# pierluigiferrari/ssd_keras

Measured on AMD Instinct MI355X. Metric: images/sec SSD300 fwd+decode @batch32, higher is better.
Workload: dtype f32 (decode, threshold, TF-style f32 NMS, top-k); bf16 conv backbone; 1 GPU; SSD300 VGG-16 inference (mode='inference': forward + DecodeDetections), 21 classes, batch 32 per GPU, conf 0.01 / NMS 0.45 / top-200, random-init weights, synthetic 300x300x3 uint8-range images; per_gpu_batch=32, global_batch=32, conv_dtype=bf16, parallelism=replicas x1, launch=hip_graph (forward + DecodeDetections captured once, replayed per step), decode_stream=same stream; DecodeDetections reads the head outputs directly (no y_pred in HBM)

## Files before the change

### ssd_keras_amd/csrc/ssdhip_conv64.hip

```cpp
#include <hip/hip_runtime.h>
#include <stdint.h>
#include <stdlib.h>

#include <type_traits>

#include "ssdhip.h"
#include "ssdhip_math.h"

#ifndef SSDHIP_C64_ABLATE
#define SSDHIP_C64_ABLATE 0
#endif

namespace ssdhip {

typedef unsigned short bf16_t;
typedef __bf16 bf16x8 __attribute__((ext_vector_type(8)));
typedef float f32x16 __attribute__((ext_vector_type(16)));
typedef int i32x4 __attribute__((ext_vector_type(4)));

#ifdef SSDHIP_PROFILE
__device__ unsigned long long g_prof64[32];
#define C64_PROF_DECL long long _pt = clock64(); long long _pa[8] = {0, 0, 0, 0, 0, 0, 0, 0}; int _pn = 0;
#define C64_PROF_MARK(i) { const long long _t = clock64(); _pa[i] += _t - _pt; _pt = _t; }
#define C64_PROF_TILE ++_pn;
#define C64_PROF_FLUSH(base) if (lane == 0) { for (int _i = 0; _i < 8; ++_i) atomicAdd(&g_prof64[(base) + _i], (unsigned long long)_pa[_i]); atomicAdd(&g_prof64[(base) + 8], (unsigned long long)_pn); }
#else
#define C64_PROF_DECL
#define C64_PROF_MARK(i)
#define C64_PROF_TILE
#define C64_PROF_FLUSH(base)
#endif

#ifndef SSDHIP_C64_NLOAD
#define SSDHIP_C64_NLOAD 1
#endif
constexpr int C64_NLOAD = SSDHIP_C64_NLOAD;
constexpr int C64_THREADS = (4 + C64_NLOAD) * 64;
constexpr int C64_NPROD = 3;
constexpr int C64_FRONT_THREADS = (4 + C64_NPROD) * 64;
constexpr int C64_WBYTES = 9 * 64 * 128;
constexpr int C64_STAGE = 0;
constexpr int c64_halo_bytes(int cs) { return ((9 * (2 * (64 >> cs) + 2) * ((1 << cs) + 2) + 63) / 64) * 1024; }
constexpr int C64_PATCH1 = 1600;
constexpr int C64_PATCH = ((C64_NPROD * C64_PATCH1 + 1023) / 1024) * 1024;
constexpr int C64_WREG_BYTES = 1024;
constexpr int c64_lds_bytes(int cs, int nb, bool front = false, bool wreg = false) {
    return (wreg ? C64_WREG_BYTES : C64_WBYTES) + nb * c64_halo_bytes(cs) + C64_STAGE + (front ? C64_PATCH : 0);
}

struct C64Params {
    const bf16_t* x;
    const bf16_t* w;
    const bf16_t* bias;
    bf16_t* y;
    int B, H, W, Cout, relu;
    int HT, WT, n_slices, tiles;
    int Ho, Wo;
    int x_bytes, w_bytes;
    const bf16_t* x3;
    const bf16_t* w1;
    const bf16_t* b1;
    int prio;
    int xcd_pairs;
    bf16_t* y2;
};

__device__ __forceinline__ u32 c64_f2bf_rn(float f) {
    const u32 u = __float_as_uint(f);
    if ((u & 0x7fffffffu) > 0x7f800000u) return (u >> 16) | 0x40u;
    return (u + 0x7fffu + ((u >> 16) & 1u)) >> 16;
}

#if defined(__HIP_DEVICE_COMPILE__)
typedef __bf16 c64_bf16x2 __attribute__((ext_vector_type(2)));
typedef float c64_f32x2 __attribute__((ext_vector_type(2)));
__device__ __forceinline__ u32 c64_pack2(float a, float b) {
    const c64_f32x2 v = {a, b};
    return __builtin_bit_cast(u32, __builtin_convertvector(v, c64_bf16x2));
}
__device__ __forceinline__ float c64_max_with_lane_xor1(float v) {
    float r;
    asm("s_nop 1\n\tv_max_f32_dpp %0, %1, %1 quad_perm:[1,0,3,2] row_mask:0xf bank_mask:0xf" : "=v"(r) : "v"(v));
    return r;
}
typedef short c64_s16x2 __attribute__((ext_vector_type(2)));
typedef u32 c64_u32x2 __attribute__((ext_vector_type(2)));
__device__ __forceinline__ u32 c64_pkmax_i16(u32 a, u32 b) {
    return __builtin_bit_cast(u32, __builtin_elementwise_max(__builtin_bit_cast(c64_s16x2, a), __builtin_bit_cast(c64_s16x2, b)));
}
typedef u32 c64_u32x4 __attribute__((ext_vector_type(4)));
__device__ __forceinline__ void c64_store_runs(const u32 (&lo)[4], const u32 (&hi)[4], __amdgpu_buffer_rsrc_t ry, u32 voff, u32 soff) {
#pragma unroll
    for (int pr = 0; pr < 2; ++pr) {
        const auto sl = __builtin_amdgcn_permlane32_swap(lo[2 * pr], lo[2 * pr + 1], false, false);
        const auto sh = __builtin_amdgcn_permlane32_swap(hi[2 * pr], hi[2 * pr + 1], false, false);
        if (!(SSDHIP_C64_ABLATE & 1)) __builtin_amdgcn_raw_buffer_store_b128(c64_u32x4{sl[0], sh[0], sl[1], sh[1]}, ry, voff + pr * 32, soff, 0);
    }
}
__device__ __forceinline__ float c64_relu(float v) { return v <= 0.f ? 0.f : v; }

__device__ __forceinline__ void c64_bload(u32 voff, i32x4 rsrc, u32 lds_dst, u32 soff = 0) {
    u32 keep;
    asm volatile("s_mov_b32 %0, m0\n\ts_mov_b32 m0, %3\n\ts_nop 0\n\tbuffer_load_dwordx4 %1, %2, %4 offen lds\n\ts_mov_b32 m0, %0"
                 : "=&s"(keep) : "v"(voff), "s"(rsrc), "s"(lds_dst), "s"(soff) : "memory");
}

__device__ __forceinline__ u32 c64_load_u16(u32 voff, i32x4 rsrc, u32 soff) {
    u32 v;
    asm volatile("buffer_load_ushort %0, %1, %2, %3 offen" : "=v"(v) : "v"(voff), "s"(rsrc), "s"(soff) : "memory");
    return v;
}

__device__ __forceinline__ i32x4 c64_rsrc(const void* base, int num_records) {
    const unsigned long long a = (unsigned long long)(uintptr_t)base;
    i32x4 r;
    r.x = (int)(u32)a;
    r.y = (int)((u32)(a >> 32) & 0xffffu);
    r.z = num_records;
    r.w = 0x00020000;
    return r;
}

template <int CS, bool POOL, int NB, bool FRONT, bool WREG, bool KEEP = false>
__device__ __forceinline__ void conv64_body(const C64Params& p, unsigned char* lds) {
    static_assert(!KEEP || (POOL && !FRONT), "KEEP is a variant of the pooled, un-fused kernel");
    constexpr int CC = 1 << CS, RP = 64 >> CS;
    constexpr int HC = CC + 2, HR = 2 * RP + 2;
    constexpr int HPX = HR * HC;
    constexpr int SLOTS = 9 * HPX;
    constexpr int NP = (SLOTS + 63) / 64;
    constexpr int HB = NP * 1024;
    static_assert(HB == c64_halo_bytes(CS) && c64_lds_bytes(CS, NB, FRONT, WREG) <= 160 * 1024, "LDS budget");
    constexpr int WB = WREG ? C64_WREG_BYTES : C64_WBYTES;
    constexpr int W_OFF = 0, H_OFF = WB, STAGE_OFF = WB + NB * HB, PATCH_OFF = STAGE_OFF + C64_STAGE;
    constexpr unsigned OOB = 0x80000000u;

    const int G = (int)gridDim.x;
    int slice = (int)blockIdx.x % p.n_slices, first = (int)blockIdx.x / p.n_slices;
    const int stride = G / p.n_slices;
    if (p.xcd_pairs) {
        const int xcd = (int)blockIdx.x & 7, j = (int)blockIdx.x >> 3;
        slice = j % p.n_slices;
        first = xcd + 8 * (j / p.n_slices);
    }
    if (first >= p.tiles) return;
    const int co0 = slice * 64;

    const int tid = threadIdx.x, lane = tid & 63;
    const int wave = __builtin_amdgcn_readfirstlane(tid >> 6);
    const int wc = wave >> 1, wp = wave & 1;
    const int r31 = lane & 31, khalf = lane >> 5;
    const u32 lds0 = (u32)(uintptr_t)(__attribute__((address_space(3))) unsigned char*)lds;
    const int xneg = (p.W + 1) * 128;
    const i32x4 rx = c64_rsrc(reinterpret_cast<const unsigned char*>(p.x) - xneg, p.x_bytes + 2 * xneg);
    const i32x4 rw = c64_rsrc(p.w, p.w_bytes);

    if (!WREG && wave < 4) {
        const int pos = lane & 7;
#pragma unroll
        for (int t = 0; t < 9; ++t)
#pragma unroll
            for (int i = 0; i < 2; ++i) {
                const int piece = i * 4 + wave;
                const int row = piece * 8 + (lane >> 3);
                const int j = pos ^ ((row >> 1) & 7);
                c64_bload((u32)((co0 + row) * 1152 + t * 128 + j * 16), rw, lds0 + W_OFF + t * 8192 + piece * 1024);
            }
    }

    auto tile_origin = [&](int tile, int& b, int& h0, int& w0) {
        const int wt = tile % p.WT, r = tile / p.WT;
        b = r / p.HT;
        h0 = (r - b * p.HT) * (2 * RP);
        w0 = wt * CC;
    };

    if constexpr (FRONT) {
      if (wave >= 4) {
        const int prod = wave - 4;
        constexpr int PR = HR + 2, PC = HC + 2, PROW = PC * 3, PATCH = PR * PROW;
        constexpr int NRAW = (PATCH + 63) / 64, NBLK = (HPX + 31) / 32, MYB = NBLK / C64_NPROD;
        static_assert(NB == 2 && (PR + 1) * PROW * 2 <= C64_PATCH1 && NRAW * 64 * 2 <= C64_PATCH1 && NBLK % C64_NPROD == 0,
                      "two halo buffers; a patch copy holds the patch, a spare row and every raw slot");
        unsigned char* patch = lds + PATCH_OFF + prod * C64_PATCH1;
        for (int i = lane; i < C64_PATCH1 / 4; i += 64) reinterpret_cast<u32*>(patch)[i] = 0u;
        bf16x8 aw[2][2];
#pragma unroll
        for (int cb = 0; cb < 2; ++cb)
#pragma unroll
            for (int st = 0; st < 2; ++st) {
                union { bf16x8 v; unsigned short u[8]; } t;
#pragma unroll
                for (int j = 0; j < 8; ++j) {
                    const int k = (2 * st + khalf) * 8 + j;
                    t.u[j] = k < 27 ? p.w1[(cb * 32 + r31) * 27 + k] : (unsigned short)0;
                }
                aw[cb][st] = t.v;
            }
        float b1v[2][16];
#pragma unroll
        for (int cb = 0; cb < 2; ++cb)
#pragma unroll
            for (int g = 0; g < 4; ++g)
#pragma unroll
                for (int e = 0; e < 4; ++e)
                    b1v[cb][4 * g + e] = p.b1 ? __uint_as_float((u32)p.b1[cb * 32 + 8 * g + 4 * khalf + e] << 16) : 0.f;
        u32 kofs[2][8];
#pragma unroll
        for (int st = 0; st < 2; ++st)
#pragma unroll
            for (int j = 0; j < 8; ++j) {
                const int k = (2 * st + khalf) * 8 + j;
                kofs[st][j] = (u32)(((k / 9) * PROW + (k % 9)) * 2);
            }
        u32 pbase[MYB], hdst[MYB], hcoord[MYB];
#pragma unroll
        for (int blk = 0; blk < MYB; ++blk) {
            const int hp = (C64_NPROD * blk + prod) * 32 + r31, hpc = hp < HPX ? hp : HPX - 1;
            const int hr = hpc / HC, hc = hpc - hr * HC;
            pbase[blk] = (u32)((hr * PROW + hc * 3) * 2);
            hdst[blk] = (u32)(hpc * 144 + 8 * khalf);
            hcoord[blk] = (u32)((hr << 8) | hc | (hp < HPX ? 0 : 0x10000));
        }
        const i32x4 r3 = c64_rsrc(p.x3, p.B * p.H * p.W * 6);
        u32 rrel[NRAW], rco[NRAW];
#pragma unroll
        for (int i = 0; i < NRAW; ++i) {
            const int n = 64 * i + lane, nn = n < PATCH ? n : 0;
            const int pr = nn / PROW, rem = nn - pr * PROW, pc = rem / 3;
            rrel[i] = n < PATCH ? (u32)(((pr * p.W) * 3 + rem) * 2) : OOB;
            rco[i] = (u32)((pr << 8) | pc);
        }
        auto request = [&](int tile, u32 (&raw)[NRAW]) {
            int b, h0, w0;
            tile_origin(tile, b, h0, w0);
            const int ph = h0 - 2, pw = w0 - 2;
            const bool inside = ph >= 0 && pw >= 0 && ph + PR <= p.H && pw + PC <= p.W;
            if (inside) {
                const u32 soff = (u32)((((b * p.H + ph) * p.W + pw) * 3) * 2);
#pragma unroll
                for (int i = 0; i < NRAW; ++i) raw[i] = c64_load_u16(rrel[i], r3, soff);
            } else {
                const int base = ((b * p.H + ph) * p.W + pw) * 6;
#pragma unroll
                for (int i = 0; i < NRAW; ++i) {
                    const int pr = (int)(rco[i] >> 8) & 0xff, pc = (int)rco[i] & 0xff;
                    const bool ok = rrel[i] != OOB && (unsigned)(ph + pr) < (unsigned)p.H && (unsigned)(pw + pc) < (unsigned)p.W;
                    raw[i] = c64_load_u16(ok ? (u32)(base + (int)rrel[i]) : OOB, r3, 0u);
                }
            }
        };
        C64_PROF_DECL
        auto landed = [&](u32 (&raw)[NRAW], bool newer) {
            if (newer) asm volatile("s_waitcnt vmcnt(%0)" :: "n"(NRAW) : "memory");
            else asm volatile("s_waitcnt vmcnt(0)" ::: "memory");
#pragma unroll
            for (int i = 0; i < NRAW; ++i) asm volatile("" : "+v"(raw[i]));
        };
        auto produce = [&](int tile, const u32 (&raw)[NRAW], int buf) {
            int b, h0, w0;
            tile_origin(tile, b, h0, w0);
#pragma unroll
            for (int i = 0; i < NRAW; ++i) reinterpret_cast<unsigned short*>(patch)[64 * i + lane] = (unsigned short)raw[i];
            unsigned char* hb = lds + H_OFF + buf * HB;
            bf16x8 bfr[MYB][2];
#pragma unroll
            for (int blk = 0; blk < MYB; ++blk)
#pragma unroll
                for (int st = 0; st < 2; ++st) {
                    union { bf16x8 v; unsigned short u[8]; } t;
#pragma unroll
                    for (int j = 0; j < 8; ++j) t.u[j] = *reinterpret_cast<const unsigned short*>(patch + pbase[blk] + kofs[st][j]);
                    bfr[blk][st] = t.v;
                }
            if (p.prio & 2) __builtin_amdgcn_s_setprio(3);
            f32x16 a1[MYB][2];
#pragma unroll
            for (int blk = 0; blk < MYB; ++blk)
#pragma unroll
                for (int cb = 0; cb < 2; ++cb) {
#pragma unroll
                    for (int v = 0; v < 16; ++v) a1[blk][cb][v] = 0.f;
                    a1[blk][cb] = __builtin_amdgcn_mfma_f32_32x32x16_bf16(aw[cb][0], bfr[blk][0], a1[blk][cb], 0, 0, 0);
                }
#pragma unroll
            for (int blk = 0; blk < MYB; ++blk)
#pragma unroll
                for (int cb = 0; cb < 2; ++cb) a1[blk][cb] = __builtin_amdgcn_mfma_f32_32x32x16_bf16(aw[cb][1], bfr[blk][1], a1[blk][cb], 0, 0, 0);
            if (p.prio & 2) __builtin_amdgcn_s_setprio(0);
            C64_PROF_MARK(2)
            auto finish = [&](auto edge) {
                constexpr bool EDGE = decltype(edge)::value;
#pragma unroll
                for (int blk = 0; blk < MYB; ++blk) {
                    const int hr = (int)(hcoord[blk] >> 8) & 0xff, hc = (int)hcoord[blk] & 0xff;
                    const bool live = (blk + 1 < MYB) || !(hcoord[blk] & 0x10000);
                    const bool in_img = !EDGE || ((unsigned)(h0 - 1 + hr) < (unsigned)p.H && (unsigned)(w0 - 1 + hc) < (unsigned)p.W);
                    const u32 keep = in_img ? 0xffffffffu : 0u;
#pragma unroll
                    for (int cb = 0; cb < 2; ++cb)
#pragma unroll
                        for (int g = 0; g < 4; ++g) {
                            float o[4];
#pragma unroll
                            for (int e = 0; e < 4; ++e) o[e] = a1[blk][cb][4 * g + e] + b1v[cb][4 * g + e];
                            u32 lo = c64_pkmax_i16(c64_pack2(o[0], o[1]), 0u), hi = c64_pkmax_i16(c64_pack2(o[2], o[3]), 0u);
                            if constexpr (EDGE) { lo &= keep; hi &= keep; }
                            if (live) *reinterpret_cast<uint2*>(hb + hdst[blk] + (cb * 32 + 8 * g) * 2) = make_uint2(lo, hi);
                        }
                }
            };
            if (h0 >= 1 && w0 >= 1 && h0 - 1 + HR <= p.H && w0 - 1 + HC <= p.W) finish(std::false_type{});
            else finish(std::true_type{});
            C64_PROF_MARK(3)
        };
        u32 raw_a[NRAW], raw_b[NRAW];
        request(first, raw_a);
        landed(raw_a, false);
        produce(first, raw_a, 0);
        if (first + stride < p.tiles) request(first + stride, raw_a);
        asm volatile("s_waitcnt lgkmcnt(0)" ::: "memory");
        __builtin_amdgcn_s_barrier();
        int buf = 0;
        auto step = [&](int tile, u32 (&cur)[NRAW], u32 (&nxt)[NRAW]) {
            const bool req = !(SSDHIP_C64_ABLATE & 8) && tile + 2 * stride < p.tiles;
            if (req) request(tile + 2 * stride, nxt);
            C64_PROF_MARK(0)
            if (!(SSDHIP_C64_ABLATE & 8) && tile + stride < p.tiles) {
                landed(cur, req);
                C64_PROF_MARK(1)
                produce(tile + stride, cur, buf ^ 1);
            }
            asm volatile("s_waitcnt lgkmcnt(0)" ::: "memory");
            C64_PROF_MARK(4)
            __builtin_amdgcn_s_barrier();
            C64_PROF_MARK(5)
            C64_PROF_TILE
            buf ^= 1;
        };
        for (int tile = first; tile < p.tiles; tile += 2 * stride) {
            step(tile, raw_a, raw_b);
            if (tile + stride >= p.tiles) break;
            step(tile + stride, raw_b, raw_a);
        }
        if (wave == 4) { C64_PROF_FLUSH(16) }
        return;
      }
    }

    if (!FRONT && wave >= 4) {
        const int lw = wave - 4;
        constexpr int NPW = NP / C64_NLOAD;
        static_assert(NP % C64_NLOAD == 0, "every loader wave issues the same number of pieces (compile-time wait counts)");
        int hrc[NPW];
        u32 rel[NPW];
#pragma unroll
        for (int k = 0; k < NPW; ++k) {
            const int n = 64 * (k * C64_NLOAD + lw) + lane;
            const int px = n / 9, c = n - 9 * px;
            const int hr = px / HC, hc = px - hr * HC;
            const bool data = c < 8 && px < HPX;
            hrc[k] = data ? ((hr << 16) | (hc << 4) | c) : -1;
            rel[k] = data ? (u32)((hr * p.W + hc) * 128 + c * 16) : OOB;
        }
        auto issue_halo = [&](int tile, int buf) {
            int b, h0, w0;
            tile_origin(tile, b, h0, w0);
            const u32 dst = lds0 + H_OFF + buf * HB + lw * 1024;
            if (h0 >= 1 && w0 >= 1 && h0 + 2 * RP + 1 <= p.H && w0 + CC + 1 <= p.W) {
                const u32 soff = (u32)(((b * p.H + h0 - 1) * p.W + (w0 - 1)) * 128 + xneg);
#pragma unroll
                for (int k = 0; k < NPW; ++k) c64_bload(rel[k], rx, dst + k * C64_NLOAD * 1024, soff);
            } else {
#pragma unroll
                for (int k = 0; k < NPW; ++k) {
                    const int h = h0 - 1 + (hrc[k] >> 16), w = w0 - 1 + ((hrc[k] >> 4) & 0xfff);
                    const bool ok = hrc[k] >= 0 && (unsigned)h < (unsigned)p.H && (unsigned)w < (unsigned)p.W;
                    const u32 voff = ok ? (u32)(((b * p.H + h) * p.W + w) * 128 + (hrc[k] & 15) * 16 + xneg) : OOB;
                    c64_bload(voff, rx, dst + k * C64_NLOAD * 1024);
                }
            }
        };
        static_assert(FRONT || (NB == 3 && 2 * NPW <= 63), "wait accounting: two halos of NPW loads in flight must fit vmcnt");
        issue_halo(first, 0);
        if (first + stride < p.tiles) issue_halo(first + stride, 1);
        if (first + 2 * stride < p.tiles) issue_halo(first + 2 * stride, 2);
        if (first + 2 * stride < p.tiles) asm volatile("s_waitcnt vmcnt(%0)" :: "n"(2 * NPW) : "memory");
        else if (first + stride < p.tiles) asm volatile("s_waitcnt vmcnt(%0)" :: "n"(NPW) : "memory");
        else asm volatile("s_waitcnt vmcnt(0)" ::: "memory");
        __builtin_amdgcn_s_barrier();
        int buf = 0;
        C64_PROF_DECL
        for (int tile = first; tile < p.tiles; tile += stride) {
            if (tile + 2 * stride < p.tiles) asm volatile("s_waitcnt vmcnt(%0)" :: "n"(NPW) : "memory");
            else asm volatile("s_waitcnt vmcnt(0)" ::: "memory");
            C64_PROF_MARK(0)
            __builtin_amdgcn_s_barrier();
            C64_PROF_MARK(1)
            if (tile + 3 * stride < p.tiles) issue_halo(tile + 3 * stride, buf);
            C64_PROF_MARK(2)
            C64_PROF_TILE
            buf = buf + 1 == NB ? 0 : buf + 1;
        }
        if (wave == 4) { C64_PROF_FLUSH(16) }
        return;
    }

    if (p.prio & 1) __builtin_amdgcn_s_setprio(2);
    const int q = wp * 32 + r31;
    const int rp = q >> CS, col = q & (CC - 1);
    u32 bbase[2];
#pragma unroll
    for (int pi = 0; pi < 2; ++pi) bbase[pi] = (u32)(H_OFF + ((2 * rp + pi) * HC + col) * 144 + khalf * 16);
    u32 ylane[2];
    [[maybe_unused]] u32 yfull[2] = {0u, 0u};
    if constexpr (KEEP) {
#pragma unroll
        for (int pi = 0; pi < 2; ++pi) yfull[pi] = (u32)((((2 * rp + pi) * p.W + col) * p.Cout) * 2 + khalf * 16);
    }
    if constexpr (POOL) {
        ylane[0] = ylane[1] = (u32)(((rp * p.Wo + (col >> 1)) * p.Cout) * 2 + khalf * 16);
    } else {
#pragma unroll
        for (int pi = 0; pi < 2; ++pi) ylane[pi] = (u32)((((2 * rp + pi) * p.W + col) * p.Cout) * 2 + khalf * 16);
    }
    u32 abase[4];
    {
        const int row = wc * 32 + r31;
#pragma unroll
        for (int kk = 0; kk < 4; ++kk) abase[kk] = (u32)(W_OFF + row * 128 + (((2 * kk + khalf) ^ ((row >> 1) & 7)) << 4));
    }
    bf16x8 wreg[WREG ? 36 : 1];
    if constexpr (WREG) {
        const bf16_t* wrow = p.w + (size_t)(co0 + wc * 32 + r31) * 576 + khalf * 8;
#pragma unroll
        for (int s = 0; s < 36; ++s) wreg[s] = *reinterpret_cast<const bf16x8*>(wrow + (s >> 2) * 64 + (s & 3) * 16);
        if (wave == 0) reinterpret_cast<float*>(lds + W_OFF)[lane] = p.bias ? __uint_as_float((u32)p.bias[co0 + lane] << 16) : 0.f;
    }
    float bv[16];
    if constexpr (!WREG) {
#pragma unroll
        for (int g = 0; g < 4; ++g)
#pragma unroll
            for (int e = 0; e < 4; ++e) {
                const int ch = co0 + wc * 32 + 8 * g + 4 * khalf + e;
                bv[4 * g + e] = p.bias ? __uint_as_float((u32)p.bias[ch] << 16) : 0.f;
            }
    }

    asm volatile("s_waitcnt vmcnt(0) lgkmcnt(0)" ::: "memory");
    if constexpr (WREG) {
#pragma unroll
        for (int s = 0; s < 36; ++s) asm volatile("" : "+v"(wreg[s]));
    }
    __builtin_amdgcn_s_barrier();

    int buf = 0;
    C64_PROF_DECL
    for (int tile = first; tile < p.tiles; tile += stride) {
        const unsigned char* hb = lds + buf * HB;

        f32x16 acc[2];
#pragma unroll
        for (int pi = 0; pi < 2; ++pi)
#pragma unroll
            for (int v = 0; v < 16; ++v) acc[pi][v] = 0.f;

        constexpr int RD = WREG ? 4 : 5, RS = RD + 1;
        bf16x8 fa[WREG ? 1 : RS], fb0[RS], fb1[RS];
        auto rd = [&](const int s, const int slot) {
            const int t = s >> 2, kk = s & 3;
            const int timm = ((t / 3) * HC + (t % 3)) * 144 + kk * 32;
            fb0[slot] = *reinterpret_cast<const bf16x8*>(hb + bbase[0] + timm);
            if constexpr (!WREG) fa[slot] = *reinterpret_cast<const bf16x8*>(lds + abase[kk] + t * 8192);
            fb1[slot] = *reinterpret_cast<const bf16x8*>(hb + bbase[1] + timm);
        };
#pragma unroll
        for (int s = 0; s < RD; ++s) rd(s, s);
        __builtin_amdgcn_sched_barrier(0);
#pragma unroll
        for (int s = 0; s < 36; ++s) {
            if ((s + RD < 36) && (!(SSDHIP_C64_ABLATE & 4) || s + RD < RS)) rd(s + RD, (s + RD) % RS);
            __builtin_amdgcn_sched_barrier(0);
            acc[1] = __builtin_amdgcn_mfma_f32_32x32x16_bf16(WREG ? wreg[WREG ? s : 0] : fa[WREG ? 0 : s % RS], fb1[s % RS], acc[1], 0, 0, 0);
            acc[0] = __builtin_amdgcn_mfma_f32_32x32x16_bf16(WREG ? wreg[WREG ? s : 0] : fa[WREG ? 0 : s % RS], fb0[s % RS], acc[0], 0, 0, 0);
            __builtin_amdgcn_sched_barrier(0);
        }

        if constexpr (WREG) {
#pragma unroll
            for (int g = 0; g < 4; ++g) {
                const float4 t4 = *reinterpret_cast<const float4*>(lds + W_OFF + (wc * 32 + 8 * g + 4 * khalf) * 4);
                bv[4 * g] = t4.x; bv[4 * g + 1] = t4.y; bv[4 * g + 2] = t4.z; bv[4 * g + 3] = t4.w;
            }
        }
        C64_PROF_MARK(0)
        __builtin_amdgcn_s_barrier();
        buf = buf + 1 == NB ? 0 : buf + 1;
        C64_PROF_MARK(1)

        int b, h0, w0;
        tile_origin(tile, b, h0, w0);
        const u32 floor16 = p.relu ? 0u : 0x80008000u;
        if constexpr ((SSDHIP_C64_ABLATE & 2) != 0) {
            asm volatile("" :: "v"(acc[0]), "v"(acc[1]));
        } else
        if constexpr (POOL) {
            if constexpr (KEEP) {
                const size_t img2 = (size_t)p.H * p.W * p.Cout * 2;
                const __amdgpu_buffer_rsrc_t ry2 = __builtin_amdgcn_make_buffer_rsrc(reinterpret_cast<unsigned char*>(p.y2) + (size_t)b * img2, 0, (int)img2, 0x00020000);
                const u32 sbase2 = (u32)(((h0 * p.W + w0) * p.Cout + co0 + wc * 32) * 2);
#pragma unroll
                for (int pi = 0; pi < 2; ++pi) {
                    const bool ok = ((h0 + 2 * rp + pi) < p.H) & ((w0 + col) < p.W);
                    const u32 voff2 = yfull[pi] | (ok ? 0u : OOB);
                    u32 lo[4], hi[4];
#pragma unroll
                    for (int g = 0; g < 4; ++g) {
                        lo[g] = c64_pkmax_i16(c64_pack2(acc[pi][4 * g] + bv[4 * g], acc[pi][4 * g + 1] + bv[4 * g + 1]), floor16);
                        hi[g] = c64_pkmax_i16(c64_pack2(acc[pi][4 * g + 2] + bv[4 * g + 2], acc[pi][4 * g + 3] + bv[4 * g + 3]), floor16);
                    }
                    c64_store_runs(lo, hi, ry2, voff2, sbase2);
                }
            }
            const size_t img = (size_t)p.Ho * p.Wo * p.Cout * 2;
            const __amdgpu_buffer_rsrc_t ry = __builtin_amdgcn_make_buffer_rsrc(reinterpret_cast<unsigned char*>(p.y) + (size_t)b * img, 0, (int)img, 0x00020000);
            const u32 sbase = (u32)((((h0 >> 1) * p.Wo + (w0 >> 1)) * p.Cout + co0 + wc * 32) * 2);
            const int hq = h0 + 2 * rp, wq = w0 + col;
            const bool okp = (!(r31 & 1)) & (((h0 >> 1) + rp) < p.Ho) & ((wq >> 1) < p.Wo);
            const u32 voff = ylane[0] | (okp ? 0u : OOB);
            auto pooled = [&](auto edge) {
                constexpr bool EDGE = decltype(edge)::value;
                const bool has_below = !EDGE || hq + 1 < p.H, has_right = !EDGE || wq + 1 < p.W;
                u32 lo[4], hi[4];
#pragma unroll
                for (int g = 0; g < 4; ++g) {
                    float o[4];
#pragma unroll
                    for (int e = 0; e < 4; ++e) {
                        float v = acc[0][4 * g + e];
                        if constexpr (EDGE) {
                            const float below = acc[1][4 * g + e];
                            if (has_below) v = below > v ? below : v;
                            const float right = __int_as_float(__builtin_amdgcn_update_dpp(0, __float_as_int(v), 0xB1, 0xf, 0xf, false));
                            if (has_right) v = right > v ? right : v;
                        } else {
                            const float below = acc[1][4 * g + e];
                            v = below > v ? below : v;
                            v = c64_max_with_lane_xor1(v);
                        }
                        o[e] = v + bv[4 * g + e];
                    }
                    lo[g] = c64_pkmax_i16(c64_pack2(o[0], o[1]), floor16);
                    hi[g] = c64_pkmax_i16(c64_pack2(o[2], o[3]), floor16);
                }
                c64_store_runs(lo, hi, ry, voff, sbase);
            };
            if (h0 + 2 * RP <= p.H && w0 + CC <= p.W) pooled(std::false_type{});
            else pooled(std::true_type{});
        } else {
            const size_t img = (size_t)p.H * p.W * p.Cout * 2;
            const __amdgpu_buffer_rsrc_t ry = __builtin_amdgcn_make_buffer_rsrc(reinterpret_cast<unsigned char*>(p.y) + (size_t)b * img, 0, (int)img, 0x00020000);
            const u32 sbase = (u32)(((h0 * p.W + w0) * p.Cout + co0 + wc * 32) * 2);
#pragma unroll
            for (int pi = 0; pi < 2; ++pi) {
                const bool ok = ((h0 + 2 * rp + pi) < p.H) & ((w0 + col) < p.W);
                const u32 voff = ylane[pi] | (ok ? 0u : OOB);
                u32 lo[4], hi[4];
#pragma unroll
                for (int g = 0; g < 4; ++g) {
                    lo[g] = c64_pkmax_i16(c64_pack2(acc[pi][4 * g] + bv[4 * g], acc[pi][4 * g + 1] + bv[4 * g + 1]), floor16);
                    hi[g] = c64_pkmax_i16(c64_pack2(acc[pi][4 * g + 2] + bv[4 * g + 2], acc[pi][4 * g + 3] + bv[4 * g + 3]), floor16);
                }
                c64_store_runs(lo, hi, ry, voff, sbase);
            }
        }
        C64_PROF_MARK(2)
        C64_PROF_TILE
    }
    if (wave == 0) { C64_PROF_FLUSH(0) }
}
#endif

template <int CS, bool POOL, int NB, bool FRONT = false, bool WREG = false, bool KEEP = false>
__global__ __launch_bounds__(FRONT ? C64_FRONT_THREADS : C64_THREADS, 1) void conv64_kernel(C64Params p) {
#if defined(__HIP_DEVICE_COMPILE__)
    __shared__ __attribute__((aligned(1024))) unsigned char lds[c64_lds_bytes(CS, NB, FRONT, WREG)];
    conv64_body<CS, POOL, NB, FRONT, WREG, KEEP>(p, lds);
#endif
}

}

using namespace ssdhip;

static int c64_launch(const void* x, const void* weight, const void* bias, void* y, void* y2, int B, int H, int W, int Cin, int Cout, int relu,
                      int pool, int n_workgroups, void* stream_) {
    hipStream_t stream = static_cast<hipStream_t>(stream_);
    if (!x || !weight || !y || B <= 0 || H <= 0 || W <= 0 || Cin != 64 || Cout <= 0 || (Cout % 64)) return SSDHIP_E_BADARG;
    if (((uintptr_t)x | (uintptr_t)weight | (uintptr_t)y | (uintptr_t)y2) & 15 || ((uintptr_t)bias & 1)) return SSDHIP_E_BADARG;
    if (y2 && !pool) return SSDHIP_E_BADARG;
    const long long xb = (long long)B * H * W * 128, wb = (long long)Cout * 1152;
    if (xb >= 0x7ffff000LL || wb >= 0x7ffff000LL || (long long)B * H * W * Cout > 0x7fffffff0LL) return SSDHIP_E_BADARG;
    C64Params p;
    p.x = static_cast<const bf16_t*>(x); p.w = static_cast<const bf16_t*>(weight); p.bias = static_cast<const bf16_t*>(bias);
    p.y = static_cast<bf16_t*>(y);
    p.B = B; p.H = H; p.W = W; p.Cout = Cout; p.relu = relu ? 1 : 0;
    p.Ho = (H + 1) / 2; p.Wo = (W + 1) / 2;
    p.x_bytes = (int)xb; p.w_bytes = (int)wb;
    p.x3 = nullptr; p.w1 = nullptr; p.b1 = nullptr;
    p.y2 = static_cast<bf16_t*>(y2);
    { const char* e = getenv("SSDHIP_C64_PRIO"); p.prio = e ? atoi(e) : 1; }
    p.n_slices = Cout / 64;
    int cs_best = 4;
    long long best = -1;
    for (int cs = 4; cs >= 3; --cs) {
        const long long wt = (W + (1 << cs) - 1) >> cs, ht = (p.Ho + (64 >> cs) - 1) / (64 >> cs);
        if (best < 0 || wt * ht < best) { best = wt * ht; cs_best = cs; p.WT = (int)wt; p.HT = (int)ht; }
    }
    const long long tiles = (long long)B * p.HT * p.WT;
    if (tiles > 0x3fffffffLL) return SSDHIP_E_BADARG;
    p.tiles = (int)tiles;
    int G = n_workgroups > 0 ? n_workgroups : 256;
    if (G > 4096) G = 4096;
    G = (G / p.n_slices) * p.n_slices;
    if (G < p.n_slices) G = p.n_slices;
    { const char* e = getenv("SSDHIP_C64_XCD"); p.xcd_pairs = (p.n_slices > 1 && G % (8 * p.n_slices) == 0 && !(e && atoi(e) == 0)) ? 1 : 0; }
    static const bool wreg = []() { const char* e = getenv("SSDHIP_C64_WREG"); return e ? atoi(e) != 0 : true; }();
#define C64_LAUNCH(CS_, POOL_) do { if (wreg) hipLaunchKernelGGL((conv64_kernel<CS_, POOL_, 3, false, true>), dim3(G), dim3(C64_THREADS), 0, stream, p); \
                                    else hipLaunchKernelGGL((conv64_kernel<CS_, POOL_, 3>), dim3(G), dim3(C64_THREADS), 0, stream, p); } while (0)
    if (pool && y2) {
        if (cs_best == 3) hipLaunchKernelGGL((conv64_kernel<3, true, 3, false, true, true>), dim3(G), dim3(C64_THREADS), 0, stream, p);
        else hipLaunchKernelGGL((conv64_kernel<4, true, 3, false, true, true>), dim3(G), dim3(C64_THREADS), 0, stream, p);
    } else if (pool) {
        if (cs_best == 3) C64_LAUNCH(3, true); else C64_LAUNCH(4, true);
    } else {
        if (cs_best == 3) C64_LAUNCH(3, false); else C64_LAUNCH(4, false);
    }
#undef C64_LAUNCH
    return hipGetLastError() == hipSuccess ? SSDHIP_OK : SSDHIP_E_LAUNCH;
}

extern "C" int ssdhip_conv3x3_c64_nhwc_bf16(const void* x, const void* weight, const void* bias, void* y, int B, int H, int W,
                                            int Cin, int Cout, int relu, int pool, int n_workgroups, void* stream) {
    return c64_launch(x, weight, bias, y, nullptr, B, H, W, Cin, Cout, relu, pool, n_workgroups, stream);
}

extern "C" int ssdhip_conv3x3_c64_pool_keep_nhwc_bf16(const void* x, const void* weight, const void* bias, void* y_full, void* y_pooled, int B,
                                                      int H, int W, int Cin, int Cout, int relu, int n_workgroups, void* stream) {
    if (!y_full) return SSDHIP_E_BADARG;
    return c64_launch(x, weight, bias, y_pooled, y_full, B, H, W, Cin, Cout, relu, 1, n_workgroups, stream);
}

extern "C" int ssdhip_conv1_block_nhwc_bf16(const void* x3, const void* w1, const void* b1, const void* weight, const void* bias, void* y,
                                            int B, int H, int W, int Cout, int relu, int pool, int n_workgroups, void* stream_) {
    hipStream_t stream = static_cast<hipStream_t>(stream_);
    if (!x3 || !w1 || !weight || !y || B <= 0 || H <= 0 || W <= 0 || Cout <= 0 || (Cout % 64)) return SSDHIP_E_BADARG;
    if (((uintptr_t)weight | (uintptr_t)y) & 15 || (((uintptr_t)x3 | (uintptr_t)w1 | (uintptr_t)b1 | (uintptr_t)bias) & 1)) return SSDHIP_E_BADARG;
    const long long wb = (long long)Cout * 1152;
    if ((long long)B * H * W * 6 >= 0x7ffff000LL || wb >= 0x7ffff000LL || (long long)B * H * W * Cout > 0x7fffffff0LL) return SSDHIP_E_BADARG;
    C64Params p;
    p.x = nullptr; p.w = static_cast<const bf16_t*>(weight); p.bias = static_cast<const bf16_t*>(bias);
    p.y = static_cast<bf16_t*>(y);
    p.x3 = static_cast<const bf16_t*>(x3); p.w1 = static_cast<const bf16_t*>(w1); p.b1 = static_cast<const bf16_t*>(b1);
    p.y2 = nullptr;
    { const char* e = getenv("SSDHIP_C64_PRIO"); p.prio = e ? atoi(e) : 3; }
    p.B = B; p.H = H; p.W = W; p.Cout = Cout; p.relu = relu ? 1 : 0;
    p.Ho = (H + 1) / 2; p.Wo = (W + 1) / 2;
    p.x_bytes = 0; p.w_bytes = (int)wb;
    p.n_slices = Cout / 64;
    int cs_best = 4;
    long long best = -1;
    for (int cs = 4; cs >= 3; --cs) {
        const long long wt = (W + (1 << cs) - 1) >> cs, ht = (p.Ho + (64 >> cs) - 1) / (64 >> cs);
        if (best < 0 || wt * ht < best) { best = wt * ht; cs_best = cs; p.WT = (int)wt; p.HT = (int)ht; }
    }
    const long long tiles = (long long)B * p.HT * p.WT;
    if (tiles > 0x3fffffffLL) return SSDHIP_E_BADARG;
    p.tiles = (int)tiles;
    int G = n_workgroups > 0 ? n_workgroups : 256;
    if (G > 4096) G = 4096;
    G = (G / p.n_slices) * p.n_slices;
    if (G < p.n_slices) G = p.n_slices;
    { const char* e = getenv("SSDHIP_C64_XCD"); p.xcd_pairs = (p.n_slices > 1 && G % (8 * p.n_slices) == 0 && !(e && atoi(e) == 0)) ? 1 : 0; }
    static const bool wreg = []() { const char* e = getenv("SSDHIP_C64_WREG"); return e ? atoi(e) != 0 : true; }();
#define C64F_LAUNCH(CS_, POOL_) do { if (wreg) hipLaunchKernelGGL((conv64_kernel<CS_, POOL_, 2, true, true>), dim3(G), dim3(C64_FRONT_THREADS), 0, stream, p); \
                                     else hipLaunchKernelGGL((conv64_kernel<CS_, POOL_, 2, true>), dim3(G), dim3(C64_FRONT_THREADS), 0, stream, p); } while (0)
    if (pool) {
        if (cs_best == 3) C64F_LAUNCH(3, true); else C64F_LAUNCH(4, true);
    } else {
        if (cs_best == 3) C64F_LAUNCH(3, false); else C64F_LAUNCH(4, false);
    }
#undef C64F_LAUNCH
    return hipGetLastError() == hipSuccess ? SSDHIP_OK : SSDHIP_E_LAUNCH;
}

#ifdef SSDHIP_PROFILE
extern "C" int ssdhip_profile_read_c64(unsigned long long* host_out, int reset) {
    if (hipMemcpyFromSymbol(host_out, HIP_SYMBOL(g_prof64), sizeof(g_prof64)) != hipSuccess) return -1;
    if (reset) { unsigned long long z[32] = {0}; if (hipMemcpyToSymbol(HIP_SYMBOL(g_prof64), z, sizeof(z)) != hipSuccess) return -1; }
    return 0;
}
#endif
```

Baseline: 16680 images/sec.

## Load first-conv patch with dwordx2 and build im2col fragments from shifted LDS copy

In the fused first-layer producer waves, interior tiles on even-width images now fetch the raw 3-channel patch with 64-bit buffer loads instead of one 16-bit load per element. The patch is stored twice in LDS, once as-is and once shifted by one element, so each bf16x8 im2col fragment can be assembled from a perm of two dwords plus three aligned dword reads rather than eight scalar ushort reads. This cuts both global load instruction count and LDS read count per tile. In exchange it adds a second patch image to LDS (larger footprint per producer), masking logic for the K padding, and separate wait counts for the narrow and wide paths.

```diff
diff --git a/ssd_keras_amd/csrc/ssdhip_conv64.hip b/ssd_keras_amd/csrc/ssdhip_conv64.hip
--- a/ssd_keras_amd/csrc/ssdhip_conv64.hip
+++ b/ssd_keras_amd/csrc/ssdhip_conv64.hip
@@ -41,7 +41,9 @@
 constexpr int C64_WBYTES = 9 * 64 * 128;
 constexpr int C64_STAGE = 0;
 constexpr int c64_halo_bytes(int cs) { return ((9 * (2 * (64 >> cs) + 2) * ((1 << cs) + 2) + 63) / 64) * 1024; }
-constexpr int C64_PATCH1 = 1600;
+constexpr int C64_PCOPY = 1600;
+constexpr int C64_PSHIFT = 1724;
+constexpr int C64_PATCH1 = C64_PSHIFT + C64_PCOPY + 4;
 constexpr int C64_PATCH = ((C64_NPROD * C64_PATCH1 + 1023) / 1024) * 1024;
 constexpr int C64_WREG_BYTES = 1024;
 constexpr int c64_lds_bytes(int cs, int nb, bool front = false, bool wreg = false) {
@@ -111,6 +113,12 @@
     return v;
 }
 
+__device__ __forceinline__ c64_u32x2 c64_load_b64(u32 voff, i32x4 rsrc, u32 soff) {
+    c64_u32x2 v;
+    asm volatile("buffer_load_dwordx2 %0, %1, %2, %3 offen" : "=v"(v) : "v"(voff), "s"(rsrc), "s"(soff) : "memory");
+    return v;
+}
+
 __device__ __forceinline__ i32x4 c64_rsrc(const void* base, int num_records) {
     const unsigned long long a = (unsigned long long)(uintptr_t)base;
     i32x4 r;
@@ -179,11 +187,12 @@
       if (wave >= 4) {
         const int prod = wave - 4;
         constexpr int PR = HR + 2, PC = HC + 2, PROW = PC * 3, PATCH = PR * PROW;
-        constexpr int NRAW = (PATCH + 63) / 64, NBLK = (HPX + 31) / 32, MYB = NBLK / C64_NPROD;
-        static_assert(NB == 2 && (PR + 1) * PROW * 2 <= C64_PATCH1 && NRAW * 64 * 2 <= C64_PATCH1 && NBLK % C64_NPROD == 0,
-                      "two halo buffers; a patch copy holds the patch, a spare row and every raw slot");
+        constexpr int NRAW = (PATCH + 63) / 64, NRAW2 = (PATCH / 2 + 63) / 64, NBLK = (HPX + 31) / 32, MYB = NBLK / C64_NPROD;
+        static_assert(NB == 2 && NBLK % C64_NPROD == 0, "two halo buffers; whole halo blocks per producer");
+        static_assert(PROW % 2 == 0 && 2 * NRAW2 <= NRAW && NRAW * 64 * 2 <= C64_PCOPY && NRAW2 * 64 * 4 <= C64_PCOPY &&
+                      ((HR + 1) * PROW + 3 * (HC - 1) + 14) * 2 <= C64_PCOPY && C64_PSHIFT >= C64_PCOPY + 2 && C64_PSHIFT % 4 == 0,
+                      "patch images: every slot, every read (the last run's masked tail included) inside an image; no overlap");
         unsigned char* patch = lds + PATCH_OFF + prod * C64_PATCH1;
-        for (int i = lane; i < C64_PATCH1 / 4; i += 64) reinterpret_cast<u32*>(patch)[i] = 0u;
         bf16x8 aw[2][2];
 #pragma unroll
         for (int cb = 0; cb < 2; ++cb)
@@ -205,25 +214,28 @@
 #pragma unroll
                 for (int e = 0; e < 4; ++e)
                     b1v[cb][4 * g + e] = p.b1 ? __uint_as_float((u32)p.b1[cb * 32 + 8 * g + 4 * khalf + e] << 16) : 0.f;
-        u32 kofs[2][8];
-#pragma unroll
-        for (int st = 0; st < 2; ++st)
-#pragma unroll
-            for (int j = 0; j < 8; ++j) {
-                const int k = (2 * st + khalf) * 8 + j;
-                kofs[st][j] = (u32)(((k / 9) * PROW + (k % 9)) * 2);
-            }
-        u32 pbase[MYB], hdst[MYB], hcoord[MYB];
+        u32 rp0[MYB][2], rp1[MYB][2], rsel[MYB][2], rrun[MYB][2], hdst[MYB], hcoord[MYB];
 #pragma unroll
         for (int blk = 0; blk < MYB; ++blk) {
             const int hp = (C64_NPROD * blk + prod) * 32 + r31, hpc = hp < HPX ? hp : HPX - 1;
             const int hr = hpc / HC, hc = hpc - hr * HC;
-            pbase[blk] = (u32)((hr * PROW + hc * 3) * 2);
+            const int e0 = hr * PROW + hc * 3;
+            auto elem = [&](int k) { return e0 + (k / 9) * PROW + k % 9; };
+#pragma unroll
+            for (int st = 0; st < 2; ++st) {
+                const int k0 = (2 * st + khalf) * 8;
+                const int a = elem(k0), b = elem(k0 + 1), x = elem(k0 + 2);
+                rp0[blk][st] = (u32)((a >> 1) * 4);
+                rp1[blk][st] = (u32)((b >> 1) * 4);
+                rsel[blk][st] = (u32)((4 + 2 * (a & 1)) | ((5 + 2 * (a & 1)) << 8) | ((2 * (b & 1)) << 16) | ((2 * (b & 1) + 1) << 24));
+                rrun[blk][st] = (u32)((x & 1) ? C64_PSHIFT + 2 * (x - 1) : 2 * x);
+            }
             hdst[blk] = (u32)(hpc * 144 + 8 * khalf);
             hcoord[blk] = (u32)((hr << 8) | hc | (hp < HPX ? 0 : 0x10000));
         }
+        const u32 keep1 = khalf ? 0xffffu : 0xffffffffu, keep23 = khalf ? 0u : 0xffffffffu;
         const i32x4 r3 = c64_rsrc(p.x3, p.B * p.H * p.W * 6);
-        u32 rrel[NRAW], rco[NRAW];
+        u32 rrel[NRAW], rco[NRAW], rrel2[NRAW2];
 #pragma unroll
         for (int i = 0; i < NRAW; ++i) {
             const int n = 64 * i + lane, nn = n < PATCH ? n : 0;
@@ -231,11 +243,27 @@
             rrel[i] = n < PATCH ? (u32)(((pr * p.W) * 3 + rem) * 2) : OOB;
             rco[i] = (u32)((pr << 8) | pc);
         }
-        auto request = [&](int tile, u32 (&raw)[NRAW]) {
+#pragma unroll
+        for (int i = 0; i < NRAW2; ++i) {
+            const int n = 64 * i + lane, pr = (2 * n) / PROW, rem = 2 * n - pr * PROW;
+            rrel2[i] = 2 * n < PATCH ? (u32)(((pr * p.W) * 3 + rem) * 2) : OOB;
+        }
+        const long long npix = (long long)p.B * p.H * p.W;
+        auto request = [&](int tile, u32 (&raw)[NRAW]) -> bool {
             int b, h0, w0;
             tile_origin(tile, b, h0, w0);
             const int ph = h0 - 2, pw = w0 - 2;
             const bool inside = ph >= 0 && pw >= 0 && ph + PR <= p.H && pw + PC <= p.W;
+            if (inside && !(p.W & 1) && ((long long)(b * p.H + ph + PR - 1) * p.W + pw + PC) < npix) {
+                const u32 soff = (u32)((((b * p.H + ph) * p.W + pw) * 3) * 2);
+#pragma unroll
+                for (int i = 0; i < NRAW2; ++i) {
+                    const c64_u32x2 v = c64_load_b64(rrel2[i], r3, soff);
+                    raw[2 * i] = v[0];
+                    raw[2 * i + 1] = v[1];
+                }
+                return true;
+            }
             if (inside) {
                 const u32 soff = (u32)((((b * p.H + ph) * p.W + pw) * 3) * 2);
 #pragma unroll
@@ -249,29 +277,46 @@
                     raw[i] = c64_load_u16(ok ? (u32)(base + (int)rrel[i]) : OOB, r3, 0u);
                 }
             }
+            return false;
         };
         C64_PROF_DECL
-        auto landed = [&](u32 (&raw)[NRAW], bool newer) {
-            if (newer) asm volatile("s_waitcnt vmcnt(%0)" :: "n"(NRAW) : "memory");
+        auto landed = [&](u32 (&raw)[NRAW], int newer) {
+            if (newer == NRAW) asm volatile("s_waitcnt vmcnt(%0)" :: "n"(NRAW) : "memory");
+            else if (newer == NRAW2) asm volatile("s_waitcnt vmcnt(%0)" :: "n"(NRAW2) : "memory");
             else asm volatile("s_waitcnt vmcnt(0)" ::: "memory");
 #pragma unroll
             for (int i = 0; i < NRAW; ++i) asm volatile("" : "+v"(raw[i]));
         };
-        auto produce = [&](int tile, const u32 (&raw)[NRAW], int buf) {
+        auto produce = [&](int tile, const u32 (&raw)[NRAW], bool wide, int buf) {
             int b, h0, w0;
             tile_origin(tile, b, h0, w0);
-#pragma unroll
-            for (int i = 0; i < NRAW; ++i) reinterpret_cast<unsigned short*>(patch)[64 * i + lane] = (unsigned short)raw[i];
+            if (wide) {
+#pragma unroll
+                for (int i = 0; i < NRAW2; ++i) {
+                    const int n = 64 * i + lane;
+                    reinterpret_cast<u32*>(patch)[n] = raw[2 * i];
+                    reinterpret_cast<u32*>(patch + C64_PSHIFT)[n] = __builtin_amdgcn_alignbit(raw[2 * i + 1], raw[2 * i], 16);
+                }
+            } else {
+#pragma unroll
+                for (int i = 0; i < NRAW; ++i) {
+                    const int n = 64 * i + lane;
+                    reinterpret_cast<unsigned short*>(patch)[n] = (unsigned short)raw[i];
+                    reinterpret_cast<unsigned short*>(patch + C64_PSHIFT - 2)[n] = (unsigned short)raw[i];
+                }
+            }
             unsigned char* hb = lds + H_OFF + buf * HB;
             bf16x8 bfr[MYB][2];
 #pragma unroll
             for (int blk = 0; blk < MYB; ++blk)
 #pragma unroll
                 for (int st = 0; st < 2; ++st) {
-                    union { bf16x8 v; unsigned short u[8]; } t;
-#pragma unroll
-                    for (int j = 0; j < 8; ++j) t.u[j] = *reinterpret_cast<const unsigned short*>(patch + pbase[blk] + kofs[st][j]);
-                    bfr[blk][st] = t.v;
+                    const u32 d0 = *reinterpret_cast<const u32*>(patch + rp0[blk][st]);
+                    const u32 d1 = *reinterpret_cast<const u32*>(patch + rp1[blk][st]);
+                    const u32* run = reinterpret_cast<const u32*>(patch + rrun[blk][st]);
+                    c64_u32x4 f = {__builtin_amdgcn_perm(d0, d1, rsel[blk][st]), run[0], run[1], run[2]};
+                    if (st == 1) { f[1] &= keep1; f[2] &= keep23; f[3] &= keep23; }
+                    bfr[blk][st] = __builtin_bit_cast(bf16x8, f);
                 }
             if (p.prio & 2) __builtin_amdgcn_s_setprio(3);
             f32x16 a1[MYB][2];
@@ -315,21 +360,21 @@
             C64_PROF_MARK(3)
         };
         u32 raw_a[NRAW], raw_b[NRAW];
-        request(first, raw_a);
-        landed(raw_a, false);
-        produce(first, raw_a, 0);
-        if (first + stride < p.tiles) request(first + stride, raw_a);
+        bool wide_a = request(first, raw_a), wide_b = false;
+        landed(raw_a, 0);
+        produce(first, raw_a, wide_a, 0);
+        if (first + stride < p.tiles) wide_a = request(first + stride, raw_a);
         asm volatile("s_waitcnt lgkmcnt(0)" ::: "memory");
         __builtin_amdgcn_s_barrier();
         int buf = 0;
-        auto step = [&](int tile, u32 (&cur)[NRAW], u32 (&nxt)[NRAW]) {
+        auto step = [&](int tile, u32 (&cur)[NRAW], bool& cur_wide, u32 (&nxt)[NRAW], bool& nxt_wide) {
             const bool req = !(SSDHIP_C64_ABLATE & 8) && tile + 2 * stride < p.tiles;
-            if (req) request(tile + 2 * stride, nxt);
+            if (req) nxt_wide = request(tile + 2 * stride, nxt);
             C64_PROF_MARK(0)
             if (!(SSDHIP_C64_ABLATE & 8) && tile + stride < p.tiles) {
-                landed(cur, req);
+                landed(cur, req ? (nxt_wide ? NRAW2 : NRAW) : 0);
                 C64_PROF_MARK(1)
-                produce(tile + stride, cur, buf ^ 1);
+                produce(tile + stride, cur, cur_wide, buf ^ 1);
             }
             asm volatile("s_waitcnt lgkmcnt(0)" ::: "memory");
             C64_PROF_MARK(4)
@@ -339,9 +384,9 @@
             buf ^= 1;
         };
         for (int tile = first; tile < p.tiles; tile += 2 * stride) {
-            step(tile, raw_a, raw_b);
+            step(tile, raw_a, wide_a, raw_b, wide_b);
             if (tile + stride >= p.tiles) break;
-            step(tile + stride, raw_b, raw_a);
+            step(tile + stride, raw_b, wide_b, raw_a, wide_a);
         }
         if (wave == 4) { C64_PROF_FLUSH(16) }
         return;
```

Result: no change. 16760 images/sec, median of 6 (+0.5%).
